# bentotten/radiation_ppo

Measured on AMD Instinct MI355X. Metric: env steps/sec (whole node) at 4096 envs; PPO iters/sec at 1/2/4/8 GPUs, higher is better.
Workload: dtype f32 policy / f64+int32 env

## Files before the change

### include/radsearch.h

```cpp
#ifndef RADSEARCH_H
#define RADSEARCH_H

#include <stddef.h>
#include <stdint.h>

#ifdef __cplusplus
extern "C" {
#endif

#define RS_ABI_VERSION 4
#define RS_OBS_DIM 11
#define RS_NUM_ACTIONS 9
#define RS_MAX_AGENTS 8
#define RS_MAX_OBS 7

typedef void* rs_stream_t;
typedef struct rs_handle rs_handle;

enum {
    RS_OK = 0,
    RS_ERR_INVALID_ARG = 1,
    RS_ERR_HIP = 2,
    RS_ERR_WORKSPACE = 3,
    RS_ERR_UNSUPPORTED = 4
};

enum {
    RS_ENVERR_ZERO_DIST = 1,
    RS_ENVERR_IDLE_STALL = 2,
    RS_ENVERR_CORRECT_CAP = 4,
    RS_ENVERR_BAD_ACTION = 8,
    RS_ENVERR_NO_PATH = 16
};

typedef struct rs_config {
    int32_t num_envs;
    int32_t num_agents;
    int32_t obstruction_count;
    int32_t enforce_grid_boundaries;
    int32_t bbox[4];
    int32_t observation_area[2];
    int32_t falloff;
    int32_t geom_group_size;
    uint32_t seed;
    uint32_t env_id_base;
    int32_t coord_noise;
    int32_t debug_spawn;
} rs_config;

typedef struct rs_info {
    uint8_t* out_of_bounds;
    int32_t* out_of_bounds_count;
    uint8_t* blocked;
    uint8_t* collision;
} rs_info;

const char* rs_strerror(int code);
int rs_abi_version(void);

size_t rs_state_bytes(const rs_config* cfg);

int rs_create(const rs_config* cfg, void* workspace, size_t workspace_bytes, rs_stream_t stream, rs_handle** out);
void rs_destroy(rs_handle* h);

int rs_state_field(rs_handle* h, const char* name, void** dev_ptr, int32_t* elem_bytes, int32_t* rows, int32_t* cols);

int rs_set_epoch_end(rs_handle* h, rs_stream_t stream);

int rs_reset(rs_handle* h, const uint8_t* mask, float* obs, float* reward, float* team, uint8_t* done,
             const rs_info* info, rs_stream_t stream);

int rs_refresh(rs_handle* h, const uint8_t* mask, const int32_t* src_xy, const int32_t* det_xy, const int32_t* intensity,
               const int32_t* bkg, const int32_t* num_obs, const int32_t* rects, float* obs, float* reward, float* team,
               uint8_t* done, const rs_info* info, rs_stream_t stream);

int rs_step(rs_handle* h, const int8_t* actions, float* obs, float* reward, float* team, uint8_t* done,
            const rs_info* info, rs_stream_t stream);

int rs_action_uniforms(rs_handle* h, float* u, rs_stream_t stream);

int rs_error_flags(rs_handle* h, rs_stream_t stream, uint32_t* flags_out);

int rs_gae(const float* rew, const float* val, const uint8_t* cut, const float* last_val, float* adv, float* ret,
           int32_t T, int32_t M, double gamma, double lam, rs_stream_t stream);

typedef struct rs_mlp_params {
    const float *w1, *b1, *w2, *b2, *w3, *b3;
} rs_mlp_params;

int rs_policy_forward(const rs_mlp_params* actor, const rs_mlp_params* critic, const float* x, int32_t M,
                      float* logits, float* value, rs_stream_t stream);

typedef struct rs_rollout_args {
    int32_t steps_per_epoch;
    int32_t steps_per_episode;
    float* obs;
    int64_t* act;
    float* logp;
    float* val;
    float* rew;
    float* last_val;
    uint8_t* cut;
    float* source_tar;
    float* cur_obs;
    double* w_count;
    double* w_mean;
    double* w_sq;
    double* w_std;
    int32_t* steps_in_ep;
    float* ep_ret;
    int32_t* done_count;
    int32_t* oob_count;
    double* ep_ret_sum;
    double* ep_len_sum;
    int32_t* ep_count;
    double* ep_ret_sq_sum;
    float* ep_ret_max;
    float* ep_ret_min;
} rs_rollout_args;

int rs_rollout(rs_handle* h, const rs_mlp_params* actor, const rs_mlp_params* critic, const rs_rollout_args* args,
               rs_stream_t stream);

typedef struct rs_ppo_batch {
    const float* x;
    const int64_t* act;
    const float* adv;
    const float* ret;
    const float* logp_old;
    const float* w;
    int32_t M;
    float clip_ratio, alpha, vf_coef;
} rs_ppo_batch;

size_t rs_ppo_grad_workspace_bytes(void);
#define RS_PPO_STATS_TAIL 16
#define RS_PPO_GRAD_FLOATS (10441 + RS_PPO_STATS_TAIL)
int rs_ppo_grad(const rs_mlp_params* actor, const rs_mlp_params* critic, const rs_ppo_batch* batch, float* grads,
                double* stats, void* workspace, const int32_t* stop_flag, rs_stream_t stream);

typedef struct rs_update_state {
    int32_t adam_step;
    int32_t stopped;
    int32_t iters;
    int32_t pad;
    double last_stats[5];
} rs_update_state;

int rs_adam_step(const rs_mlp_params* actor, const rs_mlp_params* critic, const float* grads, float* m, float* v,
                 const double* stats, rs_update_state* state, float lr, float kl_threshold, rs_stream_t stream);

int rs_ppo_update_step(const rs_mlp_params* actor, const rs_mlp_params* critic, const rs_ppo_batch* batch, float* grads,
                       double* stats, void* workspace, float* m, float* v, rs_update_state* state, float lr, float kl_threshold,
                       rs_stream_t stream);

typedef struct rs_maps rs_maps;
size_t rs_maps_state_bytes(int32_t num_envs, int32_t num_agents, int32_t steps_per_episode, int32_t map_x, int32_t map_y);
int rs_maps_create(int32_t num_envs, int32_t num_agents, int32_t steps_per_episode, int32_t map_x, int32_t map_y,
                   double resolution_accuracy, const float* visit_table, void* workspace, size_t workspace_bytes,
                   rs_stream_t stream, rs_maps** out);
void rs_maps_destroy(rs_maps* m);
int rs_maps_reset(rs_maps* m, const uint8_t* mask, rs_stream_t stream);
int rs_maps_update(rs_maps* m, rs_handle* env, const float* obs, const float* pred, const uint8_t* mask, rs_stream_t stream);
int rs_maps_stack(rs_maps* m, float* actor_stack, float* critic_stack, rs_stream_t stream);
int rs_maps_field(rs_maps* m, const char* name, void** dev_ptr, int32_t* elem_bytes, int32_t* rows, int32_t* cols);

int32_t rs_cnn_trunk_slab_row(int32_t in_channels);
// ... 154 lines not shown
```

### radiation_ppo_amd/_lib.py

```python
import ctypes as C
import os

import torch

_PKG = os.path.dirname(os.path.abspath(__file__))
LIB_PATH = os.environ.get("RS_LIB_PATH") or os.path.join(_PKG, "lib", "librs_hip.so")

RS_OBS_DIM = 11
RS_MAX_AGENTS = 8
RS_MAX_OBS = 7

ENVERR_ZERO_DIST = 1
ENVERR_IDLE_STALL = 2
ENVERR_CORRECT_CAP = 4
ENVERR_BAD_ACTION = 8
ENVERR_NO_PATH = 16


class RsConfig(C.Structure):
    _fields_ = [
        ("num_envs", C.c_int32), ("num_agents", C.c_int32), ("obstruction_count", C.c_int32),
        ("enforce_grid_boundaries", C.c_int32), ("bbox", C.c_int32 * 4), ("observation_area", C.c_int32 * 2),
        ("falloff", C.c_int32), ("geom_group_size", C.c_int32), ("seed", C.c_uint32), ("env_id_base", C.c_uint32),
        ("coord_noise", C.c_int32), ("debug_spawn", C.c_int32),
    ]


class RsCollectState(C.Structure):
    _fields_ = [("num_envs", C.c_int32), ("num_agents", C.c_int32), ("steps_per_episode", C.c_int32), ("team_reward", C.c_int32)] + [
        (n, C.c_void_p) for n in ("env_obs", "env_reward", "env_team", "env_done", "obs", "ep_ret", "steps_in_ep", "w_count", "w_mean", "w_sq",
                                  "w_std", "x", "xb", "reward_used", "over", "cut", "boot", "pf_episode", "pf_calls", "episodes_begun", "t",
                                  "env_oob", "env_src_x", "env_src_y", "done_copy", "oob_copy", "src_copy", "complete_len")]


class RsMlpParams(C.Structure):
    _fields_ = [(n, C.c_void_p) for n in ("w1", "b1", "w2", "b2", "w3", "b3")]


class RsRolloutArgs(C.Structure):
    _fields_ = [("steps_per_epoch", C.c_int32), ("steps_per_episode", C.c_int32)] + [
        (n, C.c_void_p) for n in ("obs", "act", "logp", "val", "rew", "last_val", "cut", "source_tar", "cur_obs", "w_count",
                                  "w_mean", "w_sq", "w_std", "steps_in_ep", "ep_ret", "done_count", "oob_count",
                                  "ep_ret_sum", "ep_len_sum", "ep_count", "ep_ret_sq_sum", "ep_ret_max", "ep_ret_min")]


class RsPpoBatch(C.Structure):
    _fields_ = [("x", C.c_void_p), ("act", C.c_void_p), ("adv", C.c_void_p), ("ret", C.c_void_p), ("logp_old", C.c_void_p),
                ("w", C.c_void_p), ("M", C.c_int32), ("clip_ratio", C.c_float), ("alpha", C.c_float), ("vf_coef", C.c_float)]


class RsInfo(C.Structure):
    _fields_ = [("out_of_bounds", C.c_void_p), ("out_of_bounds_count", C.c_void_p), ("blocked", C.c_void_p),
                ("collision", C.c_void_p)]


SYMBOLS = [
    ("rs_strerror", C.c_char_p, [C.c_int]),
    ("rs_abi_version", C.c_int, []),
    ("rs_state_bytes", C.c_size_t, [C.POINTER(RsConfig)]),
    ("rs_create", C.c_int, [C.POINTER(RsConfig), C.c_void_p, C.c_size_t, C.c_void_p, C.POINTER(C.c_void_p)]),
    ("rs_destroy", None, [C.c_void_p]),
    ("rs_state_field", C.c_int, [C.c_void_p, C.c_char_p, C.POINTER(C.c_void_p), C.POINTER(C.c_int32),
                                 C.POINTER(C.c_int32), C.POINTER(C.c_int32)]),
    ("rs_set_epoch_end", C.c_int, [C.c_void_p, C.c_void_p]),
    ("rs_reset", C.c_int, [C.c_void_p, C.c_void_p, C.c_void_p, C.c_void_p, C.c_void_p, C.c_void_p,
                           C.POINTER(RsInfo), C.c_void_p]),
    ("rs_refresh", C.c_int, [C.c_void_p, C.c_void_p, C.c_void_p, C.c_void_p, C.c_void_p, C.c_void_p, C.c_void_p, C.c_void_p,
                             C.c_void_p, C.c_void_p, C.c_void_p, C.c_void_p, C.POINTER(RsInfo), C.c_void_p]),
    ("rs_step", C.c_int, [C.c_void_p, C.c_void_p, C.c_void_p, C.c_void_p, C.c_void_p, C.c_void_p,
                          C.POINTER(RsInfo), C.c_void_p]),
    ("rs_action_uniforms", C.c_int, [C.c_void_p, C.c_void_p, C.c_void_p]),
    ("rs_error_flags", C.c_int, [C.c_void_p, C.c_void_p, C.POINTER(C.c_uint32)]),
    ("rs_policy_forward", C.c_int, [C.POINTER(RsMlpParams), C.POINTER(RsMlpParams), C.c_void_p, C.c_int32, C.c_void_p,
                                    C.c_void_p, C.c_void_p]),
    ("rs_rollout", C.c_int, [C.c_void_p, C.POINTER(RsMlpParams), C.POINTER(RsMlpParams), C.POINTER(RsRolloutArgs), C.c_void_p]),
    ("rs_ppo_grad_workspace_bytes", C.c_size_t, []),
    ("rs_ppo_grad", C.c_int, [C.POINTER(RsMlpParams), C.POINTER(RsMlpParams), C.POINTER(RsPpoBatch), C.c_void_p, C.c_void_p,
                              C.c_void_p, C.c_void_p, C.c_void_p]),
    ("rs_adam_step", C.c_int, [C.POINTER(RsMlpParams), C.POINTER(RsMlpParams), C.c_void_p, C.c_void_p, C.c_void_p, C.c_void_p,
                               C.c_void_p, C.c_float, C.c_float, C.c_void_p]),
    ("rs_ppo_update_step", C.c_int, [C.POINTER(RsMlpParams), C.POINTER(RsMlpParams), C.POINTER(RsPpoBatch), C.c_void_p, C.c_void_p,
                                     C.c_void_p, C.c_void_p, C.c_void_p, C.c_void_p, C.c_float, C.c_float, C.c_void_p]),
    ("rs_maps_state_bytes", C.c_size_t, [C.c_int32, C.c_int32, C.c_int32, C.c_int32, C.c_int32]),
    ("rs_maps_create", C.c_int, [C.c_int32, C.c_int32, C.c_int32, C.c_int32, C.c_int32, C.c_double, C.c_void_p, C.c_void_p,
                                 C.c_size_t, C.c_void_p, C.POINTER(C.c_void_p)]),
    ("rs_maps_destroy", None, [C.c_void_p]),
    ("rs_maps_reset", C.c_int, [C.c_void_p, C.c_void_p, C.c_void_p]),
    ("rs_maps_update", C.c_int, [C.c_void_p, C.c_void_p, C.c_void_p, C.c_void_p, C.c_void_p, C.c_void_p]),
    ("rs_maps_stack", C.c_int, [C.c_void_p, C.c_void_p, C.c_void_p, C.c_void_p]),
    ("rs_maps_field", C.c_int, [C.c_void_p, C.c_char_p, C.POINTER(C.c_void_p), C.POINTER(C.c_int32), C.POINTER(C.c_int32),
                                C.POINTER(C.c_int32)]),
    ("rs_cnn_trunk_slab_row", C.c_int32, [C.c_int32]),
    ("rs_cnn_trunk_slab_rows", C.c_int32, [C.c_int64, C.c_int32]),
    ("rs_cnn_trunk_scratch_floats", C.c_int32, [C.c_int32]),
    ("rs_cnn_trunk_forward", C.c_int, [C.c_void_p, C.c_void_p, C.c_void_p, C.c_int32, C.c_int32, C.c_int64, C.c_void_p, C.c_void_p,
                                       C.c_void_p, C.c_void_p, C.c_void_p, C.c_void_p, C.c_void_p, C.c_void_p, C.c_void_p, C.c_void_p]),
    ("rs_cnn_trunk_backward", C.c_int, [C.c_void_p, C.c_void_p, C.c_void_p, C.c_int32, C.c_int32, C.c_int64, C.c_void_p, C.c_void_p,
                                        C.c_void_p, C.c_void_p, C.c_void_p, C.c_void_p, C.c_void_p, C.c_void_p]),
    ("rs_gae", C.c_int, [C.c_void_p, C.c_void_p, C.c_void_p, C.c_void_p, C.c_void_p, C.c_void_p, C.c_int32,
                         C.c_int32, C.c_double, C.c_double, C.c_void_p]),
    ("rs_pfgru_step", C.c_int, [C.c_void_p, C.c_void_p, C.c_void_p, C.c_void_p, C.c_void_p, C.c_void_p, C.c_void_p, C.c_void_p,
                                C.c_int32, C.c_double, C.c_void_p, C.c_int32, C.c_int32, C.c_void_p]),
    ("rs_pfgru_step_recorded", C.c_int, [C.c_void_p] * 7 + [C.c_int32, C.c_double, C.c_void_p, C.c_int32, C.c_int32, C.c_void_p]),
    ("rs_pfgru_pass", C.c_int, [C.c_void_p] * 7 + [C.c_double, C.c_void_p, C.c_void_p, C.c_int32, C.c_int32, C.c_void_p]),
    ("rs_pfgru_reset", C.c_int, [C.c_void_p, C.c_void_p, C.c_void_p, C.c_void_p, C.c_void_p, C.c_void_p, C.c_int32, C.c_int32,
                                 C.c_void_p]),
    ("rs_pfgru_sized_weight_floats", C.c_int32, [C.c_int32]),
    ("rs_pfgru_sized_step", C.c_int, [C.c_void_p] * 8 + [C.c_int32, C.c_double, C.c_void_p, C.c_int32, C.c_int32, C.c_int32, C.c_void_p]),
    ("rs_pfgru_sized_pass", C.c_int, [C.c_void_p] * 7 + [C.c_double, C.c_void_p, C.c_void_p, C.c_int32, C.c_int32, C.c_int32, C.c_void_p]),
    ("rs_pfgru_sized_step_recorded", C.c_int, [C.c_void_p] * 7 + [C.c_int32, C.c_double, C.c_void_p, C.c_int32, C.c_int32, C.c_int32,
                                                                    C.c_void_p]),
    ("rs_pfgru_sized_reset", C.c_int, [C.c_void_p] * 6 + [C.c_int32, C.c_int32, C.c_int32, C.c_void_p]),
    ("rs_pfgru_draws", C.c_int, [C.c_void_p, C.c_int32, C.c_int32, C.c_void_p, C.c_void_p, C.c_void_p, C.c_void_p]),
    ("rs_pfgru_train", C.c_int, [C.c_void_p] * 15 + [C.c_int32, C.c_int32, C.c_double, C.c_double, C.c_double, C.c_double, C.c_void_p]),
    ("rs_pfgru_train_keyed", C.c_int, [C.c_void_p] * 14 + [C.c_int32, C.c_int32, C.c_double, C.c_double, C.c_double, C.c_double, C.c_void_p]),
    ("rs_rnn_policy_step", C.c_int, [C.c_void_p] * 10 + [C.c_int32, C.c_void_p]),
    ("rs_rnn_policy_step_rows", C.c_int, [C.c_void_p, C.c_void_p, C.c_int32, C.c_void_p, C.c_int32, C.c_void_p, C.c_void_p, C.c_int32, C.c_void_p,
                                          C.c_void_p, C.c_void_p, C.c_void_p, C.c_void_p, C.c_int32, C.c_void_p, C.c_int32, C.c_void_p]),
    ("rs_collect_pre", C.c_int, [C.POINTER(RsCollectState), C.c_void_p]),
    ("rs_collect_post_step", C.c_int, [C.POINTER(RsCollectState), C.c_int32, C.c_void_p]),
    ("rs_collect_post_reset", C.c_int, [C.POINTER(RsCollectState), C.c_int32, C.c_void_p]),
    ("rs_welford_update", C.c_int, [C.c_void_p] * 5 + [C.c_int64, C.c_void_p, C.c_int32, C.c_int32, C.c_void_p]),
    ("rs_welford_reset", C.c_int, [C.c_void_p] * 5 + [C.c_int32, C.c_int32, C.c_void_p]),
    ("rs_welford_standardize", C.c_int, [C.c_void_p] * 3 + [C.c_int64, C.c_void_p, C.c_int64, C.c_int32, C.c_void_p]),
    ("rs_gru_h0_reset", C.c_int, [C.c_void_p] * 4 + [C.c_double, C.c_int32, C.c_int32, C.c_void_p]),
    ("rs_epoch_stats", C.c_int, [C.c_void_p] * 13 + [C.c_int32, C.c_int32, C.c_void_p]),
    ("rs_a2c_heads_loss", C.c_int, [C.c_void_p] * 11 + [C.c_int64, C.c_double, C.c_double, C.c_void_p]),
    ("rs_actor_loss", C.c_int, [C.c_void_p] * 7 + [C.c_int64, C.c_double, C.c_void_p]),
    ("rs_cnn_trunk_prepare", C.c_int, [C.c_int32] + [C.c_void_p] * 6),
    ("rs_cnn_trunk_infer", C.c_int, [C.c_void_p, C.c_void_p, C.c_void_p, C.c_int32, C.c_int32, C.c_int64, C.c_void_p, C.c_void_p, C.c_void_p]),
    ("rs_cnn_sized_slab_row", C.c_int32, [C.c_int32]),
    ("rs_cnn_sized_slab_rows", C.c_int32, [C.c_int64, C.c_int32, C.c_int32]),
    ("rs_cnn_sized_forward", C.c_int, [C.c_void_p, C.c_void_p, C.c_void_p, C.c_int32, C.c_int32, C.c_int64, C.c_int32] + [C.c_void_p] * 9),
    ("rs_cnn_sized_infer", C.c_int, [C.c_void_p, C.c_void_p, C.c_void_p, C.c_int32, C.c_int32, C.c_int64, C.c_int32] + [C.c_void_p] * 6),
    ("rs_cnn_sized_backward", C.c_int, [C.c_void_p, C.c_void_p, C.c_void_p, C.c_int32, C.c_int32, C.c_int64, C.c_int32] + [C.c_void_p] * 6
     + [C.c_int32, C.c_void_p]),
    ("rs_cnn_head", C.c_int, [C.c_void_p] * 5 + [C.c_int32, C.c_void_p, C.c_int32, C.c_void_p, C.c_void_p, C.c_void_p, C.c_int32, C.c_void_p,
                              C.c_int32, C.c_int64, C.c_void_p, C.c_int32, C.c_void_p]),
    ("rs_store_rows", C.c_int, [C.c_void_p] * 17 + [C.c_int32, C.c_int32, C.c_int32, C.c_void_p]),
    ("rs_gru_forward", C.c_int, [C.c_void_p, C.c_void_p, C.c_void_p, C.c_void_p, C.c_void_p, C.c_void_p, C.c_int32, C.c_int32, C.c_void_p]),
    ("rs_gru_backward", C.c_int, [C.c_void_p, C.c_void_p, C.c_void_p, C.c_void_p, C.c_void_p, C.c_void_p, C.c_void_p, C.c_int32,
                                  C.c_int32, C.c_void_p]),
    ("rs_rnn_sized_weight_floats", C.c_int32, [C.c_int32, C.c_int32, C.c_int32]),
    ("rs_gru_sized_weight_floats", C.c_int32, [C.c_int32]),
    ("rs_gru_sized_gate_floats", C.c_int32, [C.c_int32]),
    ("rs_rnn_sized_step", C.c_int, [C.c_void_p, C.c_int32, C.c_int32, C.c_int32, C.c_void_p, C.c_int32, C.c_void_p, C.c_int32, C.c_void_p,
                                    C.c_void_p, C.c_int32] + [C.c_void_p] * 6 + [C.c_int32, C.c_void_p, C.c_int32, C.c_void_p]),
    ("rs_gru_sized_forward", C.c_int, [C.c_void_p] * 5 + [C.c_int32, C.c_int32, C.c_int32, C.c_void_p]),
    ("rs_gru_sized_backward", C.c_int, [C.c_void_p] * 7 + [C.c_int32, C.c_int32, C.c_int32, C.c_void_p]),
    ("rs_a2c_sized_heads_loss", C.c_int, [C.c_void_p, C.c_int32, C.c_int32, C.c_int32] + [C.c_void_p] * 10
     + [C.c_int64, C.c_double, C.c_double, C.c_void_p]),
    ("rs_gru_h0_reset_sized", C.c_int, [C.c_void_p] * 4 + [C.c_double, C.c_int32, C.c_int32, C.c_int32, C.c_void_p]),
]

_lib = None

EVENTS = None


class timed:
    def __init__(self, name: str):
        self.name = name

    def __enter__(self):
        self.ev = None
        if EVENTS is not None and not torch.cuda.is_current_stream_capturing():
            self.ev = (torch.cuda.Event(enable_timing=True), torch.cuda.Event(enable_timing=True))
            self.ev[0].record()
        return self

    def __exit__(self, *exc):
        if self.ev is not None:
            self.ev[1].record()
            EVENTS.setdefault(self.name, []).append(self.ev)
        return False


def load():
    global _lib
    if _lib is not None:
        return _lib
    if not os.path.exists(LIB_PATH):
        raise RuntimeError(
# ... 19 lines not shown
```

### radiation_ppo_amd/build.py

```python
import os
import shutil
import subprocess
import sys
from concurrent.futures import ThreadPoolExecutor

PKG = os.path.dirname(os.path.abspath(__file__))
ROOT = os.path.dirname(PKG)
CSRC = os.path.join(PKG, "csrc")
LIBDIR = os.path.join(PKG, "lib")
OBJDIR = os.path.join(LIBDIR, "obj")
LIB = os.path.join(LIBDIR, "librs_hip.so")

SOURCES = ["rs_env.hip", "rs_ppo.hip", "rs_maps.hip", "rs_cnn.hip", "rs_cnn_sized.hip", "rs_pfgru.hip", "rs_gru.hip", "rs_pfgru_train.hip", "rs_rnn_policy.hip", "rs_welford.hip", "rs_cnn_loss.hip",
           "rs_rnn_sized.hip", "rs_pfgru_sized.hip"]
CFLAGS = ["--offload-arch=gfx950", "-O3", "-std=c++17", "-fPIC", "-ffp-contract=off", "-fno-fast-math", "-Wall",
          "-Wno-unused-function"]
EXTRA_CFLAGS = {"rs_ppo.hip": ["-fno-slp-vectorize"], "rs_rnn_sized.hip": ["-mllvm", "-pragma-unroll-threshold=1000000"],
                "rs_pfgru_sized.hip": ["-mllvm", "-pragma-unroll-threshold=1000000"]}


def hipcc() -> str:
    for c in (os.environ.get("HIPCC"), shutil.which("hipcc"), "/opt/rocm/bin/hipcc"):
        if c and os.path.exists(c):
            return c
    raise RuntimeError("hipcc not found: the MI355X extension cannot be built")


def _deps():
    return [os.path.join(CSRC, f) for f in os.listdir(CSRC)] + [os.path.join(ROOT, "include", "radsearch.h"), __file__]


def _newer(target: str, deps) -> bool:
    if not os.path.exists(target):
        return True
    t = os.path.getmtime(target)
    return any(os.path.getmtime(d) > t for d in deps)


def build(force: bool = False, verbose: bool = True, defines=(), suffix: str = "") -> str:
    deps = _deps()
    lib = LIB.replace(".so", suffix + ".so")
    if not force and not _newer(lib, deps):
        return lib
    os.makedirs(OBJDIR, exist_ok=True)
    cc = hipcc()

    def compile_one(src):
        obj = os.path.join(OBJDIR, src.replace(".hip", suffix + ".o"))
        if force or _newer(obj, deps):
            cmd = [cc] + CFLAGS + EXTRA_CFLAGS.get(src, []) + ["-D" + d for d in defines] + ["-c", os.path.join(CSRC, src), "-o", obj]
            if verbose:
                print("[radiation_ppo_amd.build]", " ".join(cmd), flush=True)
            subprocess.run(cmd, check=True)
        return obj

    try:
        cpus = len(os.sched_getaffinity(0))
    except AttributeError:
        cpus = os.cpu_count() or 1
    jobs = max(1, min(len(SOURCES), cpus, int(os.environ.get("MAX_JOBS") or cpus)))
    order = sorted(SOURCES, key=lambda f: f not in ("rs_rnn_sized.hip", "rs_pfgru_sized.hip"))
    with ThreadPoolExecutor(max_workers=jobs) as ex:
        done = dict(zip(order, ex.map(compile_one, order)))
    objs = [done[f] for f in SOURCES]
    cmd = [cc, "--offload-arch=gfx950", "-shared", "-fPIC"] + objs + ["-o", lib]
    if verbose:
        print("[radiation_ppo_amd.build]", " ".join(cmd), flush=True)
    subprocess.run(cmd, check=True)
    return lib


if __name__ == "__main__":
    if "--stamps" in sys.argv:
        build(force="--force" in sys.argv, defines=["RS_K7_STAMPS"], suffix="_stamps")
    else:
        build(force="--force" in sys.argv)
```

### radiation_ppo_amd/ppo.py

```python
import ctypes as C
import os
from dataclasses import dataclass
from typing import Any, Dict, List, Optional

import torch
import torch.distributed as dist
import torch.nn as nn

from . import _lib
from .envs import RadSearchVec, gae as rs_gae_call


class FFActorCritic(nn.Module):

    def __init__(self, state_dim: int = 11, action_dim: int = 8, hidden: int = 64):
        super().__init__()
        self.actor = nn.Sequential(nn.Linear(state_dim, hidden), nn.Tanh(), nn.Linear(hidden, hidden), nn.Tanh(),
                                   nn.Linear(hidden, action_dim), nn.Softmax(dim=-1))
        self.critic = nn.Sequential(nn.Linear(state_dim, hidden), nn.Tanh(), nn.Linear(hidden, hidden), nn.Tanh(),
                                    nn.Linear(hidden, 1))

    def logits(self, x: torch.Tensor) -> torch.Tensor:
        for layer in list(self.actor)[:-1]:
            x = layer(x)
# ... 146 lines not shown

    def _na(self):
        return (self.count.shape[0], self.count.shape[1] if self.count.dim() == 2 else 1)

    @staticmethod
    def _m8(mask: Optional[torch.Tensor]):
        if mask is None:
            return None
        m = mask.contiguous()
        return m.view(torch.uint8) if m.dtype == torch.bool else m.to(torch.uint8)

    def update(self, reading: torch.Tensor, mask: Optional[torch.Tensor] = None) -> None:
        if self._hip(reading):
            r, st = self._strided(reading)
            m8 = self._m8(mask)
            n, a = self._na()
            _lib.check(_lib.load().rs_welford_update(self.count.data_ptr(), self.mean.data_ptr(), self.sq.data_ptr(), self.std.data_ptr(),
                                                     r.data_ptr(), st, None if m8 is None else m8.data_ptr(), n, a,
                                                     C.c_void_p(torch.cuda.current_stream(self.count.device).cuda_stream)), "rs_welford_update")
            return
        x = reading.double()
        count = self.count + 1
        first = count == 1
        mean_new = torch.where(first, x, self.mean + (x - self.mean) / count)
        sq_new = torch.where(first, self.sq, self.sq + (x - self.mean) * (x - mean_new))
        std_new = torch.where(first, self.std, torch.clamp(torch.sqrt(sq_new / torch.clamp(count - 1, min=1)), min=1.0))
        if mask is not None:
            m = mask.view(-1, *([1] * (x.dim() - 1))).expand_as(x)
            count = torch.where(m, count, self.count)
            mean_new = torch.where(m, mean_new, self.mean)
            sq_new = torch.where(m, sq_new, self.sq)
            std_new = torch.where(m, std_new, self.std)
        self.count.copy_(count); self.mean.copy_(mean_new); self.sq.copy_(sq_new); self.std.copy_(std_new)

    def standardize(self, reading: torch.Tensor, out: Optional[torch.Tensor] = None) -> torch.Tensor:
        if self._hip(reading):
            r, st = self._strided(reading)
            if out is None:
                out = torch.empty(self.count.shape, dtype=torch.float32, device=self.count.device)
            o, ost = self._strided(out)
            assert o.data_ptr() == out.data_ptr(), "standardize(out=...) needs a float32 view with one element stride"
            _lib.check(_lib.load().rs_welford_standardize(self.mean.data_ptr(), self.std.data_ptr(), r.data_ptr(), st, o.data_ptr(), ost,
                                                          self.count.numel(),
                                                          C.c_void_p(torch.cuda.current_stream(self.count.device).cuda_stream)),
                       "rs_welford_standardize")
            return out
        z = ((reading.double() - self.mean) / self.std).float()
        if out is not None:
            out.copy_(z)
            return out
        return z

    def reset(self, mask: torch.Tensor) -> None:
        if self._hip():
            n, a = self._na()
            m8 = self._m8(mask)
            _lib.check(_lib.load().rs_welford_reset(self.count.data_ptr(), self.mean.data_ptr(), self.sq.data_ptr(), self.std.data_ptr(),
                                                    m8.data_ptr(), n, a, C.c_void_p(torch.cuda.current_stream(self.count.device).cuda_stream)),
                       "rs_welford_reset")
            return
        m = mask.view(-1, *([1] * (self.count.dim() - 1))).expand_as(self.count)
        self.count.masked_fill_(m, 0.0); self.mean.masked_fill_(m, 0.0); self.sq.masked_fill_(m, 0.0); self.std.masked_fill_(m, 1.0)


class RolloutBuffer:

    def __init__(self, T: int, N: int, A: int, obs_dim: int, device):
        f = dict(dtype=torch.float32, device=device)
        self.T, self.N, self.A = T, N, A
        self.obs = torch.zeros(T, N, A, obs_dim, **f)
        self.act = torch.zeros(T, N, A, dtype=torch.int64, device=device)
        self.rew = torch.zeros(T, N, A, **f)
        self.val = torch.zeros(T, N, A, **f)
        self.logp = torch.zeros(T, N, A, **f)
        self.last_val = torch.zeros(T, N, A, **f)
        self.cut = torch.zeros(T, N, A, dtype=torch.uint8, device=device)
        self.source_tar = torch.zeros(T, N, 2, **f)
        self.adv = torch.zeros(T, N, A, **f)
        self.ret = torch.zeros(T, N, A, **f)

    def finish(self, gamma: float, lam: float) -> None:
        rs_gae_call(self.rew, self.val, self.cut, self.last_val, gamma, lam, adv=self.adv, ret=self.ret)

    def episode_weights(self) -> torch.Tensor:
        cut = self.cut[:, :, 0].long()
        T, N = cut.shape
        seg = torch.cumsum(cut, dim=0) - cut
        n_ep = seg[-1] + 1
        lens = torch.zeros(T, N, dtype=torch.float32, device=cut.device)
        lens.scatter_add_(0, seg, torch.ones(T, N, dtype=torch.float32, device=cut.device))
        w = 1.0 / (n_ep.unsqueeze(0).float() * lens.gather(0, seg))
        return w


@dataclass
class UpdateResult:
    stop_iteration: int
    loss_policy: float
    loss_critic: float
    loss_predictor: float
    kl_divergence: float
    Entropy: float
    ClipFrac: float
    LocLoss: float
    VarExplain: int = 0


def _world() -> int:
    return dist.get_world_size() if dist.is_available() and dist.is_initialized() else 1


class Collectives:
    count = 0

    @staticmethod
    def all_reduce_sum(t: torch.Tensor) -> None:
        Collectives.count += 1
        dist.all_reduce(t, op=dist.ReduceOp.SUM)


def reduce_grads_and_stats(params, stats: torch.Tensor) -> torch.Tensor:
    if _world() == 1:
        return stats
    ps = [p for p in params if p.grad is not None]
    hi = stats.float()
    lo = (stats - hi.double()).float()
    flat = torch.cat([p.grad.reshape(-1) for p in ps] + [hi.reshape(-1), lo.reshape(-1)])
    Collectives.all_reduce_sum(flat)
    o = 0
    for p in ps:
        p.grad.copy_(flat[o:o + p.numel()].view_as(p))
        o += p.numel()
    k = stats.numel()
    return (flat[o:o + k].double() + flat[o + k:o + 2 * k].double()).view_as(stats)


def host_read(t: torch.Tensor) -> List[float]:
    if not t.is_cuda:
        return t.tolist()
    key = (t.device, t.dtype, t.numel())
    buf = _HOST_READ.get(key)
    if buf is None:
        buf = _HOST_READ[key] = (torch.empty(t.numel(), dtype=t.dtype, pin_memory=True), torch.cuda.Event())
    host, ev = buf
    host.copy_(t.reshape(-1), non_blocking=True)
    ev.record(torch.cuda.current_stream(t.device))
    while not ev.query():
        pass
    return host.tolist()


_HOST_READ: Dict[Any, Any] = {}
_SIDE: Dict[Any, Any] = {}


def side_stream(device) -> "torch.cuda.Stream":
    dev = torch.device(device)
    key = (dev.type, dev.index if dev.index is not None else torch.cuda.current_device())
    if key not in _SIDE:
        _SIDE[key] = torch.cuda.Stream(device=dev)
    return _SIDE[key]


REFERENCE_PPO_KWARGS = frozenset({
    "observation_space", "bp_args", "steps_per_epoch", "steps_per_episode", "number_of_agents", "env_height", "actor_critic_args",
    "actor_critic_architecture", "minibatch", "train_pi_iters", "train_v_iters", "train_pfgru_iters", "actor_learning_rate",
    "critic_learning_rate", "pfgru_learning_rate", "gamma", "alpha", "clip_ratio", "target_kl", "lam", "GlobalCriticOptimizer"})
# ... 51 lines not shown
                o += p.numel()

    def update_agent(self, X: torch.Tensor, act: torch.Tensor, adv: torch.Tensor, ret: torch.Tensor,
                     logp_old: torch.Tensor, w: torch.Tensor) -> UpdateResult:
        kk = 0
        kl_reached = False
        last = None
        thr = 1.5 * self.target_kl
        if self.fused_update and X.is_cuda:
            return self._update_agent_fused(X, act, adv, ret, logp_old, w)
        while not kl_reached and kk < self.train_pi_iters:
            logp, v, ent = self.agent.evaluate(X, act)
            ratio = torch.exp(logp - logp_old)
            clip_adv = torch.clamp(ratio, 1 - self.clip_ratio, 1 + self.clip_ratio) * adv
            surr = torch.min(ratio * adv, clip_adv)
            val_loss = (w * (v - ret) ** 2).sum()
            ent_m = (w * ent).sum()
            loss = -((w * surr).sum() - 0.01 * val_loss + self.alpha * ent_m.detach())
            with torch.no_grad():
                clipped = (ratio > 1 + self.clip_ratio) | (ratio < 1 - self.clip_ratio)
                stats = torch.stack([(w * (logp_old - logp)).sum(), ent_m.detach(), (w * clipped.float()).sum(),
                                     val_loss.detach(), loss.detach()]).double()
            self.pi_optimizer.zero_grad(set_to_none=True)
            loss.backward()
            stats_h = host_read(reduce_grads_and_stats(self.agent.parameters(), stats))
            last = stats_h
            if stats_h[0] < thr:
                self.pi_optimizer.step()
            else:
                kl_reached = True
            kk += 1
        self.pi_scheduler.step()
        return UpdateResult(stop_iteration=kk, loss_policy=last[4], loss_critic=last[3], loss_predictor=0.0,
                            kl_divergence=last[0], Entropy=last[1], ClipFrac=last[2], LocLoss=0.0)

    def _update_agent_fused(self, X, act, adv, ret, logp_old, w) -> UpdateResult:
        if self._fused is None:
            self._fused = FusedPPOGrad(self.agent)
        f = self._fused
        lr = self.actor_learning_rate * (0.99 ** (self.epochs_done // 100))
        thr = 1.5 * self.target_kl
        f.begin_update()
        one_rank = _world() == 1 and not os.environ.get("RS_PPO_SPLIT_TAIL")
        for _ in range(self.train_pi_iters):
            if one_rank:
                f.step(X, act, adv, ret, logp_old, w, self.clip_ratio, self.alpha, lr=lr, kl_threshold=thr)
                continue
            stats, grads = f(X, act, adv, ret, logp_old, w, self.clip_ratio, self.alpha, use_stop_flag=True)
            if _world() > 1:
                f.allreduce()
            f.adam_step(lr, thr)
        kk, stopped, _, last = f.read_state()
        self.epochs_done += 1
        return UpdateResult(stop_iteration=kk, loss_policy=last[4], loss_critic=last[3], loss_predictor=0.0,
                            kl_divergence=last[0], Entropy=last[1], ClipFrac=last[2], LocLoss=0.0)

    def save(self, path: str) -> None:
        torch.save(self.agent.state_dict(), path)

    def load(self, path: str) -> None:
        self.agent.load_state_dict(torch.load(path, map_location=self.device, weights_only=True))

    def resume_state(self) -> Dict[str, Any]:
        st: Dict[str, Any] = dict(model=self.agent.state_dict(), epochs_done=self.epochs_done,
                                  pi_optimizer=self.pi_optimizer.state_dict(), pi_scheduler=self.pi_scheduler.state_dict())
        if self._fused is not None:
            f = self._fused
            st["fused"] = dict(m=f.m.clone(), v=f.v.clone(), adam_step=int(f.state_i32[0].item()))
        return st

    def load_resume_state(self, st: Dict[str, Any]) -> None:
        self.agent.load_state_dict(st["model"])
        self.epochs_done = int(st["epochs_done"])
        self.pi_optimizer.load_state_dict(st["pi_optimizer"])
        self.pi_scheduler.load_state_dict(st["pi_scheduler"])
        if "fused" in st:
            if self._fused is None:
                self._fused = FusedPPOGrad(self.agent)
            f = self._fused
            f.m.copy_(st["fused"]["m"]); f.v.copy_(st["fused"]["v"])
            f.state_i32[0] = int(st["fused"]["adam_step"])


def normalize_advantages(adv: torch.Tensor) -> torch.Tensor:
    n = torch.tensor([adv.numel()], dtype=torch.float64, device=adv.device)
    s = adv.double().sum().view(1)
    if _world() > 1:
        pack = torch.cat([s, n])
        Collectives.all_reduce_sum(pack)
        s, n = pack[0:1], pack[1:2]
    mean = (s / n).float()
    sq = ((adv - mean) ** 2).double().sum().view(1)
    if _world() > 1:
        Collectives.all_reduce_sum(sq)
    std = torch.sqrt(sq / n).float()
    return (adv - mean) / std


class EpochStats:

    def __init__(self, A: int, device):
        f64 = dict(dtype=torch.float64, device=device)
        self.oob = torch.zeros(A, **f64)
        self.done = torch.zeros(A, **f64)
        self.ep_cnt = torch.zeros((), **f64)
        self.ep_len = torch.zeros((), **f64)
        self.ret_sum = torch.zeros(A, **f64)
        self.ret_sq = torch.zeros(A, **f64)
        self.ret_max = torch.full((A,), float("-inf"), **f64)
        self.ret_min = torch.full((A,), float("inf"), **f64)

    def zero_(self) -> None:
        for t in (self.oob, self.done, self.ep_cnt, self.ep_len, self.ret_sum, self.ret_sq):
            t.zero_()
        self.ret_max.fill_(float("-inf")); self.ret_min.fill_(float("inf"))

    def step(self, out_of_bounds: torch.Tensor, done: torch.Tensor) -> None:
        self.oob += out_of_bounds.double().sum(dim=0)
        self.done += done.double().sum(dim=0)

    def episodes(self, ep_ret: torch.Tensor, steps_in_ep: torch.Tensor, over: torch.Tensor) -> None:
        m = over.unsqueeze(1)
        r = ep_ret.double()
        self.ret_sum += (r * m).sum(dim=0)
        self.ret_sq += (r * r * m).sum(dim=0)
        self.ret_max.copy_(torch.maximum(self.ret_max, torch.where(m, r, torch.full_like(r, float("-inf"))).max(dim=0).values))
        self.ret_min.copy_(torch.minimum(self.ret_min, torch.where(m, r, torch.full_like(r, float("inf"))).min(dim=0).values))
        self.ep_len += (steps_in_ep.double() * over).sum()
        self.ep_cnt += over.double().sum()

    def step_and_episodes(self, out_of_bounds: torch.Tensor, done: torch.Tensor, ep_ret: torch.Tensor, steps_in_ep: torch.Tensor,
                          over: torch.Tensor) -> None:
        ok = (self.oob.is_cuda and out_of_bounds.dtype == torch.uint8 and done.dtype == torch.uint8 and ep_ret.dtype == torch.float32
              and steps_in_ep.dtype == torch.int32 and over.dtype == torch.bool
              and all(t.is_contiguous() for t in (out_of_bounds, done, ep_ret, steps_in_ep, over)))
        if not ok:
            self.step(out_of_bounds, done)
            self.episodes(ep_ret, steps_in_ep, over)
            return
        N, A = ep_ret.shape
        _lib.check(_lib.load().rs_epoch_stats(out_of_bounds.data_ptr(), done.data_ptr(), ep_ret.data_ptr(), steps_in_ep.data_ptr(),
                                              over.view(torch.uint8).data_ptr(), self.oob.data_ptr(), self.done.data_ptr(),
                                              self.ep_cnt.data_ptr(), self.ep_len.data_ptr(), self.ret_sum.data_ptr(), self.ret_sq.data_ptr(),
                                              self.ret_max.data_ptr(), self.ret_min.data_ptr(), N, A,
                                              C.c_void_p(torch.cuda.current_stream(self.oob.device).cuda_stream)), "rs_epoch_stats")

    def result(self) -> Dict[str, torch.Tensor]:
        return dict(DoneCount=self.done.clone(), OutOfBound=self.oob.clone(), EpCount=self.ep_cnt.clone(), EpLenSum=self.ep_len.clone(),
                    EpRetSum=self.ret_sum.clone(), EpRetSqSum=self.ret_sq.clone(), EpRetMax=self.ret_max.clone(), EpRetMin=self.ret_min.clone())


def _welford_state(w: "DeviceWelford"):
    return dict(count=w.count.clone(), mean=w.mean.clone(), sq=w.sq.clone(), std=w.std.clone())


def _welford_load(w: "DeviceWelford", st) -> None:
    w.count.copy_(st["count"]); w.mean.copy_(st["mean"]); w.sq.copy_(st["sq"]); w.std.copy_(st["std"])


class Collector:

    def __init__(self, env: RadSearchVec, agents: Dict[int, VecAgentPPO], steps_per_epoch: int, steps_per_episode: int,
                 global_critic_flag: bool = False, standardize: bool = True):
        self.env, self.agents = env, agents
        self.T, self.L = steps_per_epoch, steps_per_episode
        self.N, self.A = env.num_envs, env.number_agents
        self.team_reward = global_critic_flag
# ... 90 lines not shown


class FusedCollector:

    def __init__(self, env: RadSearchVec, agents: Dict[int, VecAgentPPO], steps_per_epoch: int, steps_per_episode: int,
                 global_critic_flag: bool = False, standardize: bool = True):
        assert env.number_agents == 1 and len(agents) == 1 and env.num_envs % 16 == 0 and standardize
        assert not global_critic_flag
        self.env, self.agents = env, agents
        self.T, self.L, self.N, self.A = steps_per_epoch, steps_per_episode, env.num_envs, 1
        dev = env.device
        self.buf = RolloutBuffer(self.T, self.N, 1, _lib.RS_OBS_DIM, dev)
        N = self.N
        f64 = dict(dtype=torch.float64, device=dev)
        self.cur_obs = torch.zeros(N, _lib.RS_OBS_DIM, dtype=torch.float32, device=dev)
        self.w_count, self.w_mean, self.w_sq = (torch.zeros(N, **f64) for _ in range(3))
        self.w_std = torch.ones(N, **f64)
        self.steps_in_ep = torch.zeros(N, dtype=torch.int32, device=dev)
        self.ep_ret = torch.zeros(N, dtype=torch.float32, device=dev)
        self.done_count = torch.zeros(N, dtype=torch.int32, device=dev)
        self.oob_count = torch.zeros(N, dtype=torch.int32, device=dev)
        self.ep_count = torch.zeros(N, dtype=torch.int32, device=dev)
        self.ep_ret_sum = torch.zeros(N, **f64)
        self.ep_len_sum = torch.zeros(N, **f64)
        self.ep_ret_sq = torch.zeros(N, **f64)
        self.ep_ret_max = torch.zeros(N, dtype=torch.float32, device=dev)
        self.ep_ret_min = torch.zeros(N, dtype=torch.float32, device=dev)
        b = self.buf
        self._args = _lib.RsRolloutArgs(
            self.T, self.L, b.obs.data_ptr(), b.act.data_ptr(), b.logp.data_ptr(), b.val.data_ptr(), b.rew.data_ptr(),
            b.last_val.data_ptr(), b.cut.data_ptr(), b.source_tar.data_ptr(), self.cur_obs.data_ptr(),
            self.w_count.data_ptr(), self.w_mean.data_ptr(), self.w_sq.data_ptr(), self.w_std.data_ptr(),
            self.steps_in_ep.data_ptr(), self.ep_ret.data_ptr(), self.done_count.data_ptr(), self.oob_count.data_ptr(),
            self.ep_ret_sum.data_ptr(), self.ep_len_sum.data_ptr(), self.ep_count.data_ptr(),
            self.ep_ret_sq.data_ptr(), self.ep_ret_max.data_ptr(), self.ep_ret_min.data_ptr())
        self.started = False

    def start(self) -> None:
        obs, *_ = self.env.reset()
        self.cur_obs.copy_(obs[:, 0])
        st = DeviceWelford((self.N,), self.env.device)
        st.update(self.cur_obs[:, 0])
        self.w_count.copy_(st.count); self.w_mean.copy_(st.mean); self.w_sq.copy_(st.sq); self.w_std.copy_(st.std)
        self.started = True

    @torch.no_grad()
    def collect(self) -> Dict[str, torch.Tensor]:
        import ctypes as C
        if not self.started:
            self.start()
        ac = self.agents[0].agent
        pa, pc = mlp_params(ac.actor), mlp_params(ac.critic)
        with _lib.timed("rs_rollout"):
            _lib.check(self.env.lib.rs_rollout(self.env._h, C.byref(pa), C.byref(pc), C.byref(self._args), self.env._stream()),
                       "rs_rollout")
        with _lib.timed("rs_gae"):
            self.buf.finish(self.agents[0].gamma, self.agents[0].lam)
        one = lambda t: t.double().sum().view(1)
        return dict(DoneCount=one(self.done_count), OutOfBound=one(self.oob_count), EpCount=self.ep_count.double().sum(),
                    EpLenSum=self.ep_len_sum.sum(), EpRetSum=one(self.ep_ret_sum), EpRetSqSum=one(self.ep_ret_sq),
                    EpRetMax=self.ep_ret_max.double().max().view(1), EpRetMin=self.ep_ret_min.double().min().view(1))

    def update(self) -> Dict[int, UpdateResult]:
        return ppo_update_from_buffer(self)

    _RESUME = ("cur_obs", "w_count", "w_mean", "w_sq", "w_std", "steps_in_ep", "ep_ret")

    def resume_state(self) -> Dict[str, Any]:
        if not self.started:
            self.start()
        return dict(env=self.env.snapshot(), **{k: getattr(self, k).clone() for k in self._RESUME})

    def load_resume_state(self, st: Dict[str, Any]) -> None:
        if not self.started:
            self.start()
        self.env.restore(st["env"])
        for k in self._RESUME:
            getattr(self, k).copy_(st[k])


def ppo_update_from_buffer(col) -> Dict[int, UpdateResult]:
    buf = col.buf
    n_total = col.N * _world()
    w = (buf.episode_weights() / n_total).reshape(-1)
    out = {}
    for a, ag in col.agents.items():
        adv = normalize_advantages(buf.adv[:, :, a]).reshape(-1)
        X = buf.obs[:, :, a].reshape(-1, buf.obs.shape[-1])
        out[a] = ag.update_agent(X, buf.act[:, :, a].reshape(-1), adv, buf.ret[:, :, a].reshape(-1),
                                 buf.logp[:, :, a].reshape(-1), w)
    return out
```

Measured before the change: 39.95 million.

## Add HIP kernels for episode weights and advantage normalization

Replaces the torch sequence of cumsum, scatter_add and gather used for per-episode weights with a single HIP kernel that scans the cut flags per column. It also replaces the multi-op torch advantage normalization with three small HIP kernels that do a two-pass f64 reduction, used only on a single GPU. The goal is fewer kernel launches and less intermediate tensor traffic in the PPO update's prepare phase. The scan kernel re-reads cut columns per chunk, and the normalization allocates a fresh workspace on every call.

```diff
diff --git a/include/radsearch.h b/include/radsearch.h
--- a/include/radsearch.h
+++ b/include/radsearch.h
@@ -83,6 +83,10 @@
 
 int rs_gae(const float* rew, const float* val, const uint8_t* cut, const float* last_val, float* adv, float* ret,
            int32_t T, int32_t M, double gamma, double lam, rs_stream_t stream);
+
+size_t rs_normalize_workspace_bytes(void);
+int rs_episode_weights(const uint8_t* cut, int64_t cut_stride, float* w, int32_t T, int32_t N, int64_t n_total, rs_stream_t stream);
+int rs_normalize_advantages(const float* adv, int64_t adv_stride, float* adv_norm, int64_t count, void* workspace, rs_stream_t stream);
 
 typedef struct rs_mlp_params {
     const float *w1, *b1, *w2, *b2, *w3, *b3;
diff --git a/radiation_ppo_amd/_lib.py b/radiation_ppo_amd/_lib.py
--- a/radiation_ppo_amd/_lib.py
+++ b/radiation_ppo_amd/_lib.py
@@ -99,6 +99,9 @@
                                         C.c_void_p, C.c_void_p, C.c_void_p, C.c_void_p, C.c_void_p, C.c_void_p]),
     ("rs_gae", C.c_int, [C.c_void_p, C.c_void_p, C.c_void_p, C.c_void_p, C.c_void_p, C.c_void_p, C.c_int32,
                          C.c_int32, C.c_double, C.c_double, C.c_void_p]),
+    ("rs_normalize_workspace_bytes", C.c_size_t, []),
+    ("rs_episode_weights", C.c_int, [C.c_void_p, C.c_int64, C.c_void_p, C.c_int32, C.c_int32, C.c_int64, C.c_void_p]),
+    ("rs_normalize_advantages", C.c_int, [C.c_void_p, C.c_int64, C.c_void_p, C.c_int64, C.c_void_p, C.c_void_p]),
     ("rs_pfgru_step", C.c_int, [C.c_void_p, C.c_void_p, C.c_void_p, C.c_void_p, C.c_void_p, C.c_void_p, C.c_void_p, C.c_void_p,
                                 C.c_int32, C.c_double, C.c_void_p, C.c_int32, C.c_int32, C.c_void_p]),
     ("rs_pfgru_step_recorded", C.c_int, [C.c_void_p] * 7 + [C.c_int32, C.c_double, C.c_void_p, C.c_int32, C.c_int32, C.c_void_p]),
diff --git a/radiation_ppo_amd/build.py b/radiation_ppo_amd/build.py
--- a/radiation_ppo_amd/build.py
+++ b/radiation_ppo_amd/build.py
@@ -12,7 +12,7 @@
 LIB = os.path.join(LIBDIR, "librs_hip.so")
 
 SOURCES = ["rs_env.hip", "rs_ppo.hip", "rs_maps.hip", "rs_cnn.hip", "rs_cnn_sized.hip", "rs_pfgru.hip", "rs_gru.hip", "rs_pfgru_train.hip", "rs_rnn_policy.hip", "rs_welford.hip", "rs_cnn_loss.hip",
-           "rs_rnn_sized.hip", "rs_pfgru_sized.hip"]
+           "rs_rnn_sized.hip", "rs_pfgru_sized.hip", "rs_prepare.hip"]
 CFLAGS = ["--offload-arch=gfx950", "-O3", "-std=c++17", "-fPIC", "-ffp-contract=off", "-fno-fast-math", "-Wall",
           "-Wno-unused-function"]
 EXTRA_CFLAGS = {"rs_ppo.hip": ["-fno-slp-vectorize"], "rs_rnn_sized.hip": ["-mllvm", "-pragma-unroll-threshold=1000000"],
diff --git a/radiation_ppo_amd/csrc/rs_prepare.hip b/radiation_ppo_amd/csrc/rs_prepare.hip
--- /dev/null
+++ b/radiation_ppo_amd/csrc/rs_prepare.hip
@@ -0,0 +1,157 @@
+#include <hip/hip_runtime.h>
+#include <stdint.h>
+
+#include "../../include/radsearch.h"
+
+namespace {
+
+constexpr int PREP_MAX_BLOCKS = 1024;
+constexpr int PREP_STATS = 4;
+
+__global__ void __launch_bounds__(64) rs_episode_weights_kernel(const uint8_t* __restrict__ cut, long long cs, float* __restrict__ w, int T,
+                                                                int N, float inv_total, int chunk) {
+    const int n = blockIdx.x * blockDim.x + threadIdx.x;
+    const int t_lo = blockIdx.y * chunk;
+    if (n >= N || t_lo >= T) return;
+    const int t_hi = min(T, t_lo + chunk) - 1;
+    const uint8_t* __restrict__ col = cut + (long long)n * cs;
+    const long long row = (long long)N * cs;
+    int n_ep = 1;
+    for (int t0 = 0; t0 < T - 1; t0 += 16) {
+        uint8_t cc[16];
+#pragma unroll
+        for (int u = 0; u < 16; ++u) cc[u] = col[(long long)min(t0 + u, T - 1) * row];
+#pragma unroll
+        for (int u = 0; u < 16; ++u) n_ep += (t0 + u < T - 1 && cc[u] != 0) ? 1 : 0;
+    }
+    int s = 0;
+    for (int t0 = t_lo - 1; t0 >= 0; t0 -= 16) {
+        uint8_t cc[16];
+#pragma unroll
+        for (int u = 0; u < 16; ++u) cc[u] = col[(long long)max(t0 - u, 0) * row];
+        int found = -1;
+#pragma unroll
+        for (int u = 15; u >= 0; --u)
+            if (t0 - u >= 0 && cc[u] != 0) found = u;
+        if (found >= 0) { s = t0 - found + 1; break; }
+    }
+    const float fn = (float)n_ep;
+    int e = -1;
+    float wv = 0.0f;
+    for (int t = t_lo; t <= t_hi; ++t) {
+        if (t > e) {
+            if (t > t_lo) s = t;
+            e = T - 1;
+            for (int t0 = t; t0 < T - 1; t0 += 16) {
+                uint8_t cc[16];
+#pragma unroll
+                for (int u = 0; u < 16; ++u) cc[u] = col[(long long)min(t0 + u, T - 1) * row];
+                int found = -1;
+#pragma unroll
+                for (int u = 15; u >= 0; --u)
+                    if (t0 + u < T - 1 && cc[u] != 0) found = u;
+                if (found >= 0) { e = t0 + found; break; }
+            }
+            wv = (1.0f / (fn * (float)(e - s + 1))) * inv_total;
+        }
+        w[(size_t)t * N + n] = wv;
+    }
+}
+
+__device__ __forceinline__ double prep_wave_sum(double v) {
+#pragma unroll
+    for (int s = 32; s >= 1; s >>= 1) v += __shfl_xor(v, s);
+    return v;
+}
+
+__device__ __forceinline__ double prep_block_sum(double v, double* red) {
+    const int lane = threadIdx.x & 63, wave = threadIdx.x >> 6;
+    v = prep_wave_sum(v);
+    if (lane == 0) red[wave] = v;
+    __syncthreads();
+    return (red[0] + red[1]) + (red[2] + red[3]);
+}
+
+__device__ __forceinline__ double prep_total(const double* __restrict__ part, int nb, double* slot) {
+    if (threadIdx.x < 64) {
+        double v = 0.0;
+        for (int j = threadIdx.x; j < nb; j += 64) v += part[j];
+        v = prep_wave_sum(v);
+        if (threadIdx.x == 0) *slot = v;
+    }
+    __syncthreads();
+    return *slot;
+}
+
+__global__ void __launch_bounds__(256) rs_adv_sum_kernel(const float* __restrict__ adv, long long st, long long M, double* __restrict__ ws) {
+    __shared__ double red[4];
+    double acc = 0.0;
+    for (long long i = (long long)blockIdx.x * 256 + threadIdx.x; i < M; i += (long long)gridDim.x * 256) acc += (double)adv[i * st];
+    const double b = prep_block_sum(acc, red);
+    if (threadIdx.x == 0) ws[PREP_STATS + blockIdx.x] = b;
+}
+
+__global__ void __launch_bounds__(256) rs_adv_sq_kernel(const float* __restrict__ adv, long long st, long long M, double n,
+                                                        double* __restrict__ ws) {
+    __shared__ double red[4];
+    __shared__ double tot;
+    const double s = prep_total(ws + PREP_STATS, gridDim.x, &tot);
+    const float mean = (float)(s / n);
+    double acc = 0.0;
+    for (long long i = (long long)blockIdx.x * 256 + threadIdx.x; i < M; i += (long long)gridDim.x * 256) {
+        const float d = adv[i * st] - mean;
+        acc += (double)(d * d);
+    }
+    const double b = prep_block_sum(acc, red);
+    if (threadIdx.x == 0) {
+        ws[PREP_STATS + PREP_MAX_BLOCKS + blockIdx.x] = b;
+        if (blockIdx.x == 0) { ws[0] = s; ws[2] = (double)mean; }
+    }
+}
+
+__global__ void __launch_bounds__(256) rs_adv_write_kernel(const float* __restrict__ adv, long long st, long long M, double n,
+                                                           double* __restrict__ ws, int nb, float* __restrict__ out) {
+    __shared__ double tot;
+    const double q = prep_total(ws + PREP_STATS + PREP_MAX_BLOCKS, nb, &tot);
+    const float mean = (float)ws[2];
+    const float sd = (float)sqrt(q / n);
+    const long long i = (long long)blockIdx.x * 256 + threadIdx.x;
+    if (i < M) out[i] = (adv[i * st] - mean) / sd;
+    if (blockIdx.x == 0 && threadIdx.x == 0) { ws[1] = q; ws[3] = (double)sd; }
+}
+
+}
+
+extern "C" {
+
+size_t rs_normalize_workspace_bytes(void) { return sizeof(double) * (PREP_STATS + 2 * PREP_MAX_BLOCKS); }
+
+int rs_episode_weights(const uint8_t* cut, int64_t cut_stride, float* w, int32_t T, int32_t N, int64_t n_total, rs_stream_t stream) {
+    if (!cut || !w || cut_stride < 1 || T < 1 || N < 1 || n_total < 1) return RS_ERR_INVALID_ARG;
+    const int col_waves = (N + 63) / 64;
+    int chunks = (512 + col_waves - 1) / col_waves;
+    chunks = chunks < 1 ? 1 : (chunks > 16 ? 16 : chunks);
+    int chunk = (T + chunks - 1) / chunks;
+    if (chunk < 32) chunk = 32;
+    chunks = (T + chunk - 1) / chunk;
+    hipLaunchKernelGGL(rs_episode_weights_kernel, dim3(col_waves, chunks), dim3(64), 0, static_cast<hipStream_t>(stream), cut,
+                       (long long)cut_stride, w, T, N, 1.0f / (float)n_total, chunk);
+    return hipGetLastError() == hipSuccess ? RS_OK : RS_ERR_HIP;
+}
+
+int rs_normalize_advantages(const float* adv, int64_t adv_stride, float* adv_norm, int64_t count, void* workspace, rs_stream_t stream) {
+    if (!adv || !adv_norm || !workspace || adv_stride < 1 || count < 1 || (reinterpret_cast<uintptr_t>(workspace) & 7)) return RS_ERR_INVALID_ARG;
+    hipStream_t s = static_cast<hipStream_t>(stream);
+    double* ws = static_cast<double*>(workspace);
+    const long long blocks = (count + 255) / 256;
+    const int nb = (int)(blocks < PREP_MAX_BLOCKS ? blocks : PREP_MAX_BLOCKS);
+    if (blocks > 0x7fffffffLL) return RS_ERR_INVALID_ARG;
+    const double n = (double)count;
+    hipLaunchKernelGGL(rs_adv_sum_kernel, dim3(nb), dim3(256), 0, s, adv, (long long)adv_stride, (long long)count, ws);
+    hipLaunchKernelGGL(rs_adv_sq_kernel, dim3(nb), dim3(256), 0, s, adv, (long long)adv_stride, (long long)count, n, ws);
+    hipLaunchKernelGGL(rs_adv_write_kernel, dim3((unsigned)blocks), dim3(256), 0, s, adv, (long long)adv_stride, (long long)count, n, ws, nb,
+                       adv_norm);
+    return hipGetLastError() == hipSuccess ? RS_OK : RS_ERR_HIP;
+}
+
+}
diff --git a/radiation_ppo_amd/ppo.py b/radiation_ppo_amd/ppo.py
--- a/radiation_ppo_amd/ppo.py
+++ b/radiation_ppo_amd/ppo.py
@@ -252,7 +252,13 @@
     def finish(self, gamma: float, lam: float) -> None:
         rs_gae_call(self.rew, self.val, self.cut, self.last_val, gamma, lam, adv=self.adv, ret=self.ret)
 
-    def episode_weights(self) -> torch.Tensor:
+    def episode_weights(self, n_total: int = 1) -> torch.Tensor:
+        if _prepare_hip(self.cut):
+            return episode_weights_hip(self.cut[:, :, 0], n_total)
+        w = self._episode_weights_torch()
+        return w if n_total == 1 else w / n_total
+
+    def _episode_weights_torch(self) -> torch.Tensor:
         cut = self.cut[:, :, 0].long()
         T, N = cut.shape
         seg = torch.cumsum(cut, dim=0) - cut
@@ -470,7 +476,53 @@
             f.state_i32[0] = int(st["fused"]["adam_step"])
 
 
+PREPARE_IMPL = os.environ.get("RS_PPO_PREPARE", "hip")
+
+
+def _prepare_hip(t: torch.Tensor) -> bool:
+    assert PREPARE_IMPL in ("hip", "torch"), PREPARE_IMPL
+    return t.is_cuda and PREPARE_IMPL == "hip"
+
+
+def _one_stride(t: torch.Tensor) -> Optional[int]:
+    dims = [(n, s) for n, s in zip(t.shape, t.stride()) if n != 1]
+    if not dims:
+        return 1
+    for (_, s0), (n1, s1) in zip(dims, dims[1:]):
+        if s0 != n1 * s1:
+            return None
+    return dims[-1][1] if dims[-1][1] >= 1 else None
+
+
+def episode_weights_hip(cut: torch.Tensor, n_total: int = 1, out: Optional[torch.Tensor] = None) -> torch.Tensor:
+    assert cut.dim() == 2 and cut.dtype == torch.uint8 and cut.is_cuda
+    st = _one_stride(cut)
+    if st is None:
+        cut, st = cut.contiguous(), 1
+    T, N = cut.shape
+    w = torch.empty(T, N, dtype=torch.float32, device=cut.device) if out is None else out
+    assert w.shape == (T, N) and w.dtype == torch.float32 and w.is_contiguous()
+    _lib.check(_lib.load().rs_episode_weights(cut.data_ptr(), st, w.data_ptr(), T, N, int(n_total),
+                                              C.c_void_p(torch.cuda.current_stream(cut.device).cuda_stream)), "rs_episode_weights")
+    return w
+
+
+def normalize_advantages_hip(adv: torch.Tensor, with_stats: bool = False):
+    assert adv.dtype == torch.float32 and adv.is_cuda and adv.numel() >= 1
+    st = _one_stride(adv)
+    if st is None:
+        adv, st = adv.contiguous(), 1
+    lib = _lib.load()
+    out = torch.empty(adv.shape, dtype=torch.float32, device=adv.device)
+    ws = torch.empty(lib.rs_normalize_workspace_bytes() // 8, dtype=torch.float64, device=adv.device)
+    _lib.check(lib.rs_normalize_advantages(adv.data_ptr(), st, out.data_ptr(), adv.numel(), ws.data_ptr(),
+                                           C.c_void_p(torch.cuda.current_stream(adv.device).cuda_stream)), "rs_normalize_advantages")
+    return (out, ws[:4]) if with_stats else out
+
+
 def normalize_advantages(adv: torch.Tensor) -> torch.Tensor:
+    if _world() == 1 and adv.dtype == torch.float32 and adv.numel() >= 1 and _prepare_hip(adv):
+        return normalize_advantages_hip(adv)
     n = torch.tensor([adv.numel()], dtype=torch.float64, device=adv.device)
     s = adv.double().sum().view(1)
     if _world() > 1:
@@ -727,7 +779,7 @@
 def ppo_update_from_buffer(col) -> Dict[int, UpdateResult]:
     buf = col.buf
     n_total = col.N * _world()
-    w = (buf.episode_weights() / n_total).reshape(-1)
+    w = buf.episode_weights(n_total).reshape(-1)
     out = {}
     for a, ag in col.agents.items():
         adv = normalize_advantages(buf.adv[:, :, a]).reshape(-1)
```

After: 39.81 million. Within noise of the previous version (-0.4%).
